# songweige/rich-text-to-image

Measured on NVIDIA H100. Metric: denoising steps/sec, higher is better.
Workload: dtype f16

## Files before the change

### include/rtti_b200.h

```cpp
#ifndef RTTI_B200_H
#define RTTI_B200_H

#ifdef __cplusplus
extern "C" {
#endif

#define RTTI_OK 0
#define RTTI_ERR_ARG (-1)
#define RTTI_ERR_SHAPE (-2)
#define RTTI_ERR_ALIGN (-3)
#define RTTI_ERR_ARCH (-4)
#define RTTI_ERR_CUDA (-5)

int rtti_version(void);
int rtti_arch_ok(void);

int rtti_attn_fwd(const void* q, const void* k, const void* v, void* o, int batch, int heads, int head_dim,
                  int n_q, int n_k, long long q_bs, long long q_rs, long long k_bs, long long k_rs,
                  long long v_bs, long long v_rs, long long o_bs, long long o_rs, float scale,
                  const int* qk_src, const int* word_pos, const float* font_size, int n_fs,
                  unsigned long long fs_batch_mask, float* pbar_accum, const int* cap_slot, float* lse,
                  void* stream);

int rtti_attn_probs_mean_accum(const void* q, const void* k, const float* lse, float* accum, int heads,
                               int head_dim, int n_q, int n_k, long long q_rs, long long k_rs, float scale,
                               void* stream);

long long rtti_groupnorm_workspace_elems(int batch, int hw, int c, int groups);
int rtti_groupnorm_silu_fwd(const void* x, const void* chan_bias, const void* gamma, const void* beta, void* y,
                            float* workspace, int batch, int hw, int c, int groups, float eps, int apply_silu,
                            void* stream);

int rtti_add_bias_f16(const void* a, const void* b, const void* bias, void* out, long long rows, int c, void* stream);

int rtti_layernorm_fwd(const void* x, const void* gamma, const void* beta, void* y, int rows, int c, float eps,
                       void* stream);

int rtti_ff_geglu_fwd(const void* x, const void* w, const void* bias, void* y, long long m, int n, int k, void* stream);

int rtti_add_bias_layernorm_fwd(const void* a, const void* resid, const void* bias, const void* gamma, const void* beta,
                                void* h_out, void* y, int rows, int c, float eps, void* stream);

int rtti_geglu_fwd(const void* proj, void* y, int rows, int inner, void* stream);

int rtti_region_blend_cfg(const void* eps_uncond, const void* const* eps_region, const float* masks,
                          int n_regions, long long n, float guidance, void* eps_out, const void* latents,
                          void* latents_out, float dt_sigma, void* stream);

long long rtti_color_loss_workspace_elems(int n_colors, long long hw);
int rtti_color_loss_fwd_bwd(const float* decoded, const float* masks, const float* target_rgb, int n_colors,
                            long long hw, float* loss_out, float* grad_decoded, float* workspace, void* stream);

int rtti_latent_guidance_update(const void* latents, const float* grad, const float* atten_all, float weight,
                                void* latents_out, long long n, void* stream);

int rtti_bg_inject_blend(const void* latents, const void* latents_ref, const float* mask, void* out,
                         long long n, void* stream);

int rtti_predict_x0(const void* x_t, const void* eps, float alpha, void* x0, long long n, void* stream);

long long rtti_gn32_workspace_elems(int batch, int hw, int c, int groups);
int rtti_gn32_silu_fwd(const float* x, const float* chan_bias, const float* gamma, const float* beta, float* y,
                       float* mean_rstd, float* workspace, int batch, int hw, int c, int groups, float eps,
                       int apply_silu, void* stream);
int rtti_gn32_silu_bwd(const float* x, const float* chan_bias, const float* dz, const float* gamma, const float* beta,
                       const float* mean_rstd, float* dx, float* workspace, int batch, int hw, int c, int groups,
                       int apply_silu, void* stream);
int rtti_add_bias_f32(const float* a, const float* b, const float* bias, float* out, long long rows, int c,
                      void* stream);

int rtti_gather_blend_step(const void* const* peer_slots, void* const* peer_flags, int world, int rank,
                           const int* slot_owner, int n_slots, int n_regions, const float* masks, long long n,
                           float guidance, void* eps_out, const void* latents, void* latents_out,
                           const void* latents_ref, void* latents_ref_out, float dt_sigma, unsigned int step_id,
                           void* stream);

int rtti_gn32_silu_fwd_striped(const float* x, const float* chan_bias, const float* gamma, const float* beta, float* y,
                               float* mean_rstd, float* workspace, int hw_local, long long hw_total, int c, int groups,
                               float eps, int apply_silu, void* const* peer_sums, void* const* peer_flags, int world,
                               int rank, unsigned int seq, void* stream);
int rtti_gn32_silu_bwd_striped(const float* x, const float* chan_bias, const float* dz, const float* gamma,
                               const float* beta, const float* mean_rstd, float* dx, float* workspace, int hw_local,
                               long long hw_total, int c, int groups, int apply_silu, void* const* peer_sums,
                               void* const* peer_flags, int world, int rank, unsigned int seq, void* stream);
int rtti_halo_exchange(float* pad_local, float* pad_up, float* pad_down, int rows, long long row_elems,
                       void* flags_local, void* flags_up, void* flags_down, unsigned int seq, void* stream);
int rtti_peer_seq_advance(void* flags_a, unsigned int da, void* flags_b, unsigned int db, void* stream);

int rtti_peer_push(const void* src, long long src_row_stride_bytes, int rows, int row_bytes, void* const* dst,
                   void* const* dst_flags, int n_dst, void* flags_local, unsigned int seq, void* stream);
int rtti_peer_wait(void* flags_local, unsigned int seq, void* stream);

#ifdef __cplusplus
}
#endif
#endif
```

### rich-text-to-image_b200/_lib.py

```python
import ctypes
import os

PKG_DIR = os.path.dirname(os.path.abspath(__file__))
LIB_PATH = os.path.join(PKG_DIR, "librtti_b200.so")

RTTI_OK = 0
_ERRORS = {
    -1: "RTTI_ERR_ARG (null pointer / out-of-range argument)",
    -2: "RTTI_ERR_SHAPE (unsupported shape)",
    -3: "RTTI_ERR_ALIGN (pointer or stride alignment)",
    -4: "RTTI_ERR_ARCH (device is not sm_90)",
    -5: "RTTI_ERR_CUDA (CUDA runtime/driver error)",
}

c_void_p, c_int, c_ll, c_float, c_ull = ctypes.c_void_p, ctypes.c_int, ctypes.c_longlong, ctypes.c_float, ctypes.c_ulonglong
P_int = ctypes.POINTER(ctypes.c_int)

SIGNATURES = {
    "rtti_version": (c_int, []),
    "rtti_arch_ok": (c_int, []),
    "rtti_attn_fwd": (c_int, [c_void_p] * 4 + [c_int] * 5 + [c_ll] * 8 + [c_float, P_int, c_void_p, c_void_p, c_int,
                                                                         c_ull, c_void_p, P_int, c_void_p, c_void_p]),
    "rtti_attn_probs_mean_accum": (c_int, [c_void_p] * 4 + [c_int] * 4 + [c_ll] * 2 + [c_float, c_void_p]),
    "rtti_groupnorm_workspace_elems": (c_ll, [c_int] * 4),
    "rtti_groupnorm_silu_fwd": (c_int, [c_void_p] * 6 + [c_int] * 4 + [c_float, c_int, c_void_p]),
    "rtti_add_bias_f16": (c_int, [c_void_p] * 4 + [c_ll, c_int, c_void_p]),
    "rtti_layernorm_fwd": (c_int, [c_void_p] * 4 + [c_int, c_int, c_float, c_void_p]),
    "rtti_add_bias_layernorm_fwd": (c_int, [c_void_p] * 7 + [c_int, c_int, c_float, c_void_p]),
    "rtti_ff_geglu_fwd": (c_int, [c_void_p] * 4 + [c_ll, c_int, c_int, c_void_p]),
    "rtti_geglu_fwd": (c_int, [c_void_p, c_void_p, c_int, c_int, c_void_p]),
    "rtti_region_blend_cfg": (c_int, [c_void_p, ctypes.POINTER(c_void_p), c_void_p, c_int, c_ll, c_float, c_void_p,
                                      c_void_p, c_void_p, c_float, c_void_p]),
    "rtti_color_loss_workspace_elems": (c_ll, [c_int, c_ll]),
    "rtti_color_loss_fwd_bwd": (c_int, [c_void_p] * 3 + [c_int, c_ll] + [c_void_p] * 4),
    "rtti_latent_guidance_update": (c_int, [c_void_p] * 3 + [c_float, c_void_p, c_ll, c_void_p]),
    "rtti_bg_inject_blend": (c_int, [c_void_p] * 4 + [c_ll, c_void_p]),
    "rtti_predict_x0": (c_int, [c_void_p, c_void_p, c_float, c_void_p, c_ll, c_void_p]),
    "rtti_gn32_workspace_elems": (c_ll, [c_int] * 4),
    "rtti_gn32_silu_fwd": (c_int, [c_void_p] * 7 + [c_int] * 4 + [c_float, c_int, c_void_p]),
    "rtti_gn32_silu_bwd": (c_int, [c_void_p] * 8 + [c_int] * 4 + [c_int, c_void_p]),
    "rtti_add_bias_f32": (c_int, [c_void_p] * 4 + [c_ll, c_int, c_void_p]),
    "rtti_gather_blend_step": (c_int, [ctypes.POINTER(c_void_p), ctypes.POINTER(c_void_p), c_int, c_int, P_int, c_int, c_int,
                                       c_void_p, c_ll, c_float, c_void_p, c_void_p, c_void_p, c_void_p, c_void_p, c_float,
                                       ctypes.c_uint, c_void_p]),
    "rtti_gn32_silu_fwd_striped": (c_int, [c_void_p] * 7 + [c_int, c_ll, c_int, c_int, c_float, c_int,
                                           ctypes.POINTER(c_void_p), ctypes.POINTER(c_void_p), c_int, c_int, ctypes.c_uint,
                                           c_void_p]),
    "rtti_gn32_silu_bwd_striped": (c_int, [c_void_p] * 8 + [c_int, c_ll, c_int, c_int, c_int,
                                           ctypes.POINTER(c_void_p), ctypes.POINTER(c_void_p), c_int, c_int, ctypes.c_uint,
                                           c_void_p]),
    "rtti_halo_exchange": (c_int, [c_void_p] * 3 + [c_int, c_ll] + [c_void_p] * 3 + [ctypes.c_uint, c_void_p]),
    "rtti_peer_seq_advance": (c_int, [c_void_p, ctypes.c_uint, c_void_p, ctypes.c_uint, c_void_p]),
    "rtti_peer_push": (c_int, [c_void_p, c_ll, c_int, c_int, ctypes.POINTER(c_void_p), ctypes.POINTER(c_void_p), c_int,
                               c_void_p, ctypes.c_uint, c_void_p]),
    "rtti_peer_wait": (c_int, [c_void_p, ctypes.c_uint, c_void_p]),
}

_lib = None


class RttiError(RuntimeError):
    pass


def load():
    global _lib
    if _lib is not None:
        return _lib
    if not os.path.exists(LIB_PATH):
        raise RttiError(
            f"{LIB_PATH} not found: build it with `python -c 'import __graft_entry__ as g; g.build()'` "
            "(the rtti_b200 product path has no CPU/PyTorch fallback)")
    lib = ctypes.CDLL(LIB_PATH)
    for name, (res, args) in SIGNATURES.items():
        fn = getattr(lib, name)
        fn.restype = res
        fn.argtypes = args
    _lib = lib
    return lib


def check(rc, what):
    if rc != RTTI_OK:
        raise RttiError(f"{what} failed: {_ERRORS.get(rc, rc)}")
```

### rich-text-to-image_b200/csrc/vae_kernels.cu

```cuda
#include "peer_sync.cuh"
#include "rtti_internal.h"

namespace rtti {

struct GN32Plan { int nvec, rowlanes, threads, chunks, rows_per_chunk; };

static GN32Plan gn32_plan(int batch, int hw, int c) {
  GN32Plan p;
  p.nvec = c / 4;
  p.rowlanes = p.nvec >= 256 ? 1 : (256 / p.nvec);
  p.threads = p.nvec * p.rowlanes;
  int want = (132 * 8 + batch - 1) / batch;
  int maxc = (hw + p.rowlanes * 8 - 1) / (p.rowlanes * 8);
  if (maxc < 1) maxc = 1;
  p.chunks = want < maxc ? want : maxc;
  if (p.chunks < 1) p.chunks = 1;
  p.rows_per_chunk = (hw + p.chunks - 1) / p.chunks;
  p.rows_per_chunk = ((p.rows_per_chunk + p.rowlanes - 1) / p.rowlanes) * p.rowlanes;
  p.chunks = (hw + p.rows_per_chunk - 1) / p.rows_per_chunk;
  return p;
}

__device__ __forceinline__ float sigmoidf_(float x) { return 1.f / (1.f + __expf(-x)); }

// ... 65 lines not shown
  }
#pragma unroll
  for (int i = 0; i < 4; ++i) {
    sm[((size_t)rl * c + vec * 4 + i) * 2] = a[i];
    sm[((size_t)rl * c + vec * 4 + i) * 2 + 1] = q[i];
  }
  __syncthreads();
  for (int g = threadIdx.x; g < groups; g += blockDim.x) {
    float s0 = 0.f, s1 = 0.f;
    for (int l = 0; l < rowlanes; ++l)
      for (int ch = g * cpg; ch < (g + 1) * cpg; ++ch) {
        s0 += sm[((size_t)l * c + ch) * 2];
        s1 += sm[((size_t)l * c + ch) * 2 + 1];
      }
    float* o = ws + (((size_t)b * chunks + chunk) * groups + g) * 2;
    o[0] = s0; o[1] = s1;
  }
}

template <int MODE>
__global__ void gn32_finalize_kernel(const float* __restrict__ ws, float* __restrict__ out, int groups, int chunks,
                                     float n, float eps) {
  const int b = blockIdx.y;
  const int g = blockIdx.x * (blockDim.x >> 5) + (threadIdx.x >> 5);
  const int lane = threadIdx.x & 31;
  if (g >= groups) return;
  float s0 = 0.f, s1 = 0.f;
  for (int k = lane; k < chunks; k += 32) {
    const float* o = ws + (((size_t)b * chunks + k) * groups + g) * 2;
    s0 += o[0]; s1 += o[1];
  }
#pragma unroll
  for (int o = 16; o > 0; o >>= 1) {
    s0 += __shfl_xor_sync(0xffffffffu, s0, o);
    s1 += __shfl_xor_sync(0xffffffffu, s1, o);
  }
  if (lane == 0) {
    float* d = out + ((size_t)b * groups + g) * 2;
    if (MODE == 0) {
      const float mean = s0 / n;
      const float var = fmaxf(s1 / n - mean * mean, 0.f);
      d[0] = mean; d[1] = rsqrtf(var + eps);
    } else {
      d[0] = s0 / n; d[1] = s1 / n;
    }
  }
}

template <int MODE>
__global__ void gn32_apply_kernel(const float* __restrict__ x, const float* __restrict__ cbias,
                                  const float* __restrict__ dz,
                                  const float* __restrict__ gamma, const float* __restrict__ beta,
                                  const float* __restrict__ mean_rstd, const float* __restrict__ c12,
                                  float* __restrict__ out, int hw, int c, int groups, int nvec, int rowlanes,
                                  int rows_per_chunk, int silu) {
  const int b = blockIdx.y, chunk = blockIdx.x;
  const int vec = threadIdx.x % nvec, rl = threadIdx.x / nvec;
  const int cpg = c / groups;
  float ga[4], be[4], mu[4], rs[4], c1[4], c2[4];
  float cb[4] = {0.f, 0.f, 0.f, 0.f};
  if (cbias) { const float4 c4 = *reinterpret_cast<const float4*>(cbias + vec * 4); cb[0] = c4.x; cb[1] = c4.y; cb[2] = c4.z; cb[3] = c4.w; }
  const float4 g4 = *reinterpret_cast<const float4*>(gamma + vec * 4);
  const float4 b4 = *reinterpret_cast<const float4*>(beta + vec * 4);
  ga[0] = g4.x; ga[1] = g4.y; ga[2] = g4.z; ga[3] = g4.w;
  be[0] = b4.x; be[1] = b4.y; be[2] = b4.z; be[3] = b4.w;
#pragma unroll
  for (int i = 0; i < 4; ++i) {
    const int g = (vec * 4 + i) / cpg;
    mu[i] = mean_rstd[((size_t)b * groups + g) * 2];
    rs[i] = mean_rstd[((size_t)b * groups + g) * 2 + 1];
    if (MODE == 1) { c1[i] = c12[((size_t)b * groups + g) * 2]; c2[i] = c12[((size_t)b * groups + g) * 2 + 1]; }
  }
  const int r0 = chunk * rows_per_chunk, r1 = min(hw, r0 + rows_per_chunk);
  const size_t base = ((size_t)b * hw) * c + vec * 4;
  auto apply = [&](const float4& xv, const float4& dv) -> float4 {
    const float xs[4] = {xv.x + cb[0], xv.y + cb[1], xv.z + cb[2], xv.w + cb[3]};
    float o[4];
    if (MODE == 0) {
#pragma unroll
      for (int i = 0; i < 4; ++i) {
        const float y = fmaf((xs[i] - mu[i]) * rs[i], ga[i], be[i]);
        o[i] = silu ? y * sigmoidf_(y) : y;
      }
    } else {
      const float ds[4] = {dv.x, dv.y, dv.z, dv.w};
#pragma unroll
      for (int i = 0; i < 4; ++i) {
        const float xh = (xs[i] - mu[i]) * rs[i];
        float dy = ds[i];
        if (silu) {
          const float y = fmaf(xh, ga[i], be[i]);
          const float s = sigmoidf_(y);
          dy *= s * (1.f + y * (1.f - s));
        }
        o[i] = rs[i] * (dy * ga[i] - c1[i] - xh * c2[i]);
      }
    }
    return make_float4(o[0], o[1], o[2], o[3]);
  };
  int r = r0 + rl;
  for (; r + 3 * rowlanes < r1; r += 4 * rowlanes) {
    float4 xv[4], dv[4];
#pragma unroll
    for (int u = 0; u < 4; ++u) {
      xv[u] = *reinterpret_cast<const float4*>(x + base + (size_t)(r + u * rowlanes) * c);
      if (MODE == 1) dv[u] = *reinterpret_cast<const float4*>(dz + base + (size_t)(r + u * rowlanes) * c);
    }
#pragma unroll
    for (int u = 0; u < 4; ++u)
      *reinterpret_cast<float4*>(out + base + (size_t)(r + u * rowlanes) * c) = apply(xv[u], dv[u]);
  }
  for (; r < r1; r += rowlanes) {
    const float4 xv = *reinterpret_cast<const float4*>(x + base + (size_t)r * c);
    float4 dv = xv;
    if (MODE == 1) dv = *reinterpret_cast<const float4*>(dz + base + (size_t)r * c);
    *reinterpret_cast<float4*>(out + base + (size_t)r * c) = apply(xv, dv);
  }
}

static int gn32_check(const void* a, const void* b_, const void* c_, const void* d, int batch, int hw, int c, int groups) {
  if (!a || !b_ || !c_ || !d) return RTTI_ERR_ARG;
  if (batch < 1 || hw < 1 || groups < 1) return RTTI_ERR_ARG;
  if (c % 4 != 0 || c % groups != 0 || c / 4 > 1024) return RTTI_ERR_SHAPE;
  if (((uintptr_t)a | (uintptr_t)b_ | (uintptr_t)c_ | (uintptr_t)d) & 15) return RTTI_ERR_ALIGN;
  return RTTI_OK;
}

struct PeerSums {
  float* sums[PEER_MAX_WORLD];
  unsigned int* flags[PEER_MAX_WORLD];
  int world, rank;
  unsigned int seq;
};

template <int MODE>
__global__ void __launch_bounds__(1024) gn32_finalize_peer_kernel(const float* __restrict__ ws, float* __restrict__ out,
                                                                  const PeerSums pp, int groups, int chunks,
                                                                  float n_total, float eps) {
  const int g = threadIdx.x >> 5, lane = threadIdx.x & 31;
  const unsigned int seq = pp.seq + *reinterpret_cast<const volatile unsigned int*>(pp.flags[pp.rank] + 8);
  const int par = (int)(seq & 1u);
  if (g < groups) {
    float s0 = 0.f, s1 = 0.f;
    for (int k = lane; k < chunks; k += 32) {
      const float* o = ws + ((size_t)k * groups + g) * 2;
      s0 += o[0]; s1 += o[1];
    }
#pragma unroll
    for (int o = 16; o > 0; o >>= 1) {
      s0 += __shfl_xor_sync(0xffffffffu, s0, o);
      s1 += __shfl_xor_sync(0xffffffffu, s1, o);
    }
    if (lane == 0) {
      float* mine = pp.sums[pp.rank] + (size_t)par * 2 * groups;
      mine[2 * g] = s0; mine[2 * g + 1] = s1;
    }
  }
  __syncthreads();
  if (threadIdx.x == 0) {
    __threadfence_system();
    st_release_sys(pp.flags[pp.rank], seq);
  }
  if (threadIdx.x < pp.world && threadIdx.x != pp.rank) {
    if (!wait_seq(pp.flags[threadIdx.x], seq)) pp.flags[pp.rank][1] = 0xDEADu;
  }
  __syncthreads();
  if (g < groups && lane == 0) {
    float t0 = 0.f, t1 = 0.f;
    for (int r = 0; r < pp.world; ++r) {
// ... 1 lines not shown
      t0 += ld_volatile_f32(p + 2 * g);
      t1 += ld_volatile_f32(p + 2 * g + 1);
    }
    float* d = out + (size_t)g * 2;
    if (MODE == 0) {
      const float mean = t0 / n_total;
      const float var = fmaxf(t1 / n_total - mean * mean, 0.f);
      d[0] = mean; d[1] = rsqrtf(var + eps);
    } else {
      d[0] = t0 / n_total; d[1] = t1 / n_total;
    }
  }
}

static int fill_peer_sums(PeerSums& pp, void* const* peer_sums, void* const* peer_flags, int world, int rank,
                          unsigned int seq) {
  if (!peer_sums || !peer_flags) return RTTI_ERR_ARG;
  if (world < 1 || world > PEER_MAX_WORLD || rank < 0 || rank >= world) return RTTI_ERR_ARG;
  for (int r = 0; r < world; ++r) {
    if (!peer_sums[r] || !peer_flags[r]) return RTTI_ERR_ARG;
    if (((uintptr_t)peer_sums[r] | (uintptr_t)peer_flags[r]) & 3) return RTTI_ERR_ALIGN;
    pp.sums[r] = (float*)peer_sums[r];
    pp.flags[r] = (unsigned int*)peer_flags[r];
  }
  pp.world = world; pp.rank = rank; pp.seq = seq;
  return RTTI_OK;
}

}

using namespace rtti;

extern "C" long long rtti_gn32_workspace_elems(int batch, int hw, int c, int groups) {
  if (batch < 1 || hw < 1 || c < 4 || groups < 1) return 0;
  const GN32Plan p = gn32_plan(batch, hw, c);
  return (long long)batch * p.chunks * groups * 2 + (long long)batch * groups * 2;
}

extern "C" int rtti_gn32_silu_fwd(const float* x, const float* chan_bias, const float* gamma, const float* beta, float* y, float* mean_rstd,
                                  float* workspace, int batch, int hw, int c, int groups, float eps, int apply_silu,
                                  void* stream) {
  int rc = gn32_check(x, gamma, beta, y, batch, hw, c, groups);
  if (rc != RTTI_OK) return rc;
  if (!mean_rstd || !workspace) return RTTI_ERR_ARG;
  const GN32Plan p = gn32_plan(batch, hw, c);
  const size_t smem = (size_t)p.rowlanes * c * 2 * sizeof(float);
  if (smem > 48 * 1024) return RTTI_ERR_SHAPE;
  cudaStream_t st = (cudaStream_t)stream;
  dim3 grid(p.chunks, batch);
  gn32_partial_kernel<0><<<grid, p.threads, smem, st>>>(x, chan_bias, nullptr, gamma, beta, nullptr, workspace, hw, c, groups,
                                                        p.nvec, p.rowlanes, p.rows_per_chunk, p.chunks, 0);
  gn32_finalize_kernel<0><<<dim3((groups + 7) / 8, batch), 256, 0, st>>>(workspace, mean_rstd, groups, p.chunks,
                                                                         (float)hw * (float)(c / groups), eps);
  gn32_apply_kernel<0><<<grid, p.threads, 0, st>>>(x, chan_bias, nullptr, gamma, beta, mean_rstd, nullptr, y, hw, c, groups,
                                                   p.nvec, p.rowlanes, p.rows_per_chunk, apply_silu);
  return cudaGetLastError() == cudaSuccess ? RTTI_OK : RTTI_ERR_CUDA;
}

extern "C" int rtti_gn32_silu_bwd(const float* x, const float* chan_bias, const float* dz, const float* gamma, const float* beta,
                                  const float* mean_rstd, float* dx, float* workspace, int batch, int hw, int c,
                                  int groups, int apply_silu, void* stream) {
  int rc = gn32_check(x, gamma, beta, dx, batch, hw, c, groups);
  if (rc != RTTI_OK) return rc;
  if (!dz || !mean_rstd || !workspace || ((uintptr_t)dz & 15)) return RTTI_ERR_ARG;
  const GN32Plan p = gn32_plan(batch, hw, c);
  const size_t smem = (size_t)p.rowlanes * c * 2 * sizeof(float);
  if (smem > 48 * 1024) return RTTI_ERR_SHAPE;
  cudaStream_t st = (cudaStream_t)stream;
  dim3 grid(p.chunks, batch);
  float* c12 = workspace + (size_t)batch * p.chunks * groups * 2;
  gn32_partial_kernel<1><<<grid, p.threads, smem, st>>>(x, chan_bias, dz, gamma, beta, mean_rstd, workspace, hw, c, groups, p.nvec,
                                                        p.rowlanes, p.rows_per_chunk, p.chunks, apply_silu);
  gn32_finalize_kernel<1><<<dim3((groups + 7) / 8, batch), 256, 0, st>>>(workspace, c12, groups, p.chunks,
                                                                         (float)hw * (float)(c / groups), 0.f);
  gn32_apply_kernel<1><<<grid, p.threads, 0, st>>>(x, chan_bias, dz, gamma, beta, mean_rstd, c12, dx, hw, c, groups, p.nvec,
                                                   p.rowlanes, p.rows_per_chunk, apply_silu);
  return cudaGetLastError() == cudaSuccess ? RTTI_OK : RTTI_ERR_CUDA;
}


extern "C" int rtti_gn32_silu_fwd_striped(const float* x, const float* chan_bias, const float* gamma, const float* beta,
                                          float* y, float* mean_rstd, float* workspace, int hw_local, long long hw_total,
                                          int c, int groups, float eps, int apply_silu, void* const* peer_sums,
                                          void* const* peer_flags, int world, int rank, unsigned int seq, void* stream) {
  int rc = gn32_check(x, gamma, beta, y, 1, hw_local, c, groups);
  if (rc != RTTI_OK) return rc;
  if (!mean_rstd || !workspace || hw_total < hw_local) return RTTI_ERR_ARG;
  if (groups > 32) return RTTI_ERR_SHAPE;
  PeerSums pp{};
  rc = fill_peer_sums(pp, peer_sums, peer_flags, world, rank, seq);
  if (rc != RTTI_OK) return rc;
  const GN32Plan p = gn32_plan(1, hw_local, c);
  const size_t smem = (size_t)p.rowlanes * c * 2 * sizeof(float);
  if (smem > 48 * 1024) return RTTI_ERR_SHAPE;
  cudaStream_t st = (cudaStream_t)stream;
  dim3 grid(p.chunks, 1);
  gn32_partial_kernel<0><<<grid, p.threads, smem, st>>>(x, chan_bias, nullptr, gamma, beta, nullptr, workspace, hw_local, c,
                                                        groups, p.nvec, p.rowlanes, p.rows_per_chunk, p.chunks, 0);
  gn32_finalize_peer_kernel<0><<<1, 32 * groups, 0, st>>>(workspace, mean_rstd, pp, groups, p.chunks,
                                                          (float)hw_total * (float)(c / groups), eps);
  gn32_apply_kernel<0><<<grid, p.threads, 0, st>>>(x, chan_bias, nullptr, gamma, beta, mean_rstd, nullptr, y, hw_local, c,
                                                   groups, p.nvec, p.rowlanes, p.rows_per_chunk, apply_silu);
  return cudaGetLastError() == cudaSuccess ? RTTI_OK : RTTI_ERR_CUDA;
}

extern "C" int rtti_gn32_silu_bwd_striped(const float* x, const float* chan_bias, const float* dz, const float* gamma,
                                          const float* beta, const float* mean_rstd, float* dx, float* workspace,
                                          int hw_local, long long hw_total, int c, int groups, int apply_silu,
                                          void* const* peer_sums, void* const* peer_flags, int world, int rank,
                                          unsigned int seq, void* stream) {
  int rc = gn32_check(x, gamma, beta, dx, 1, hw_local, c, groups);
  if (rc != RTTI_OK) return rc;
  if (!dz || !mean_rstd || !workspace || ((uintptr_t)dz & 15) || hw_total < hw_local) return RTTI_ERR_ARG;
  if (groups > 32) return RTTI_ERR_SHAPE;
  PeerSums pp{};
  rc = fill_peer_sums(pp, peer_sums, peer_flags, world, rank, seq);
  if (rc != RTTI_OK) return rc;
  const GN32Plan p = gn32_plan(1, hw_local, c);
  const size_t smem = (size_t)p.rowlanes * c * 2 * sizeof(float);
  if (smem > 48 * 1024) return RTTI_ERR_SHAPE;
  cudaStream_t st = (cudaStream_t)stream;
  dim3 grid(p.chunks, 1);
  float* c12 = workspace + (size_t)p.chunks * groups * 2;
  gn32_partial_kernel<1><<<grid, p.threads, smem, st>>>(x, chan_bias, dz, gamma, beta, mean_rstd, workspace, hw_local, c,
                                                        groups, p.nvec, p.rowlanes, p.rows_per_chunk, p.chunks, apply_silu);
  gn32_finalize_peer_kernel<1><<<1, 32 * groups, 0, st>>>(workspace, c12, pp, groups, p.chunks,
                                                          (float)hw_total * (float)(c / groups), 0.f);
  gn32_apply_kernel<1><<<grid, p.threads, 0, st>>>(x, chan_bias, dz, gamma, beta, mean_rstd, c12, dx, hw_local, c, groups,
                                                   p.nvec, p.rowlanes, p.rows_per_chunk, apply_silu);
  return cudaGetLastError() == cudaSuccess ? RTTI_OK : RTTI_ERR_CUDA;
}

__global__ void add_bias_f32_kernel(const float* __restrict__ a, const float* __restrict__ b,
                                    const float* __restrict__ bias, float* __restrict__ out, long long nvec, int cvec) {
  for (long long i = (long long)blockIdx.x * blockDim.x + threadIdx.x; i < nvec; i += (long long)gridDim.x * blockDim.x) {
    const float4 x = reinterpret_cast<const float4*>(a)[i];
    const float4 y = reinterpret_cast<const float4*>(b)[i];
    float4 z = make_float4(0.f, 0.f, 0.f, 0.f);
    if (bias) z = reinterpret_cast<const float4*>(bias)[i % cvec];
    reinterpret_cast<float4*>(out)[i] = make_float4(x.x + y.x + z.x, x.y + y.y + z.y, x.z + y.z + z.z, x.w + y.w + z.w);
  }
}

extern "C" int rtti_add_bias_f32(const float* a, const float* b, const float* bias, float* out, long long rows, int c,
                                 void* stream) {
  if (!a || !b || !out || rows < 1 || c < 4) return RTTI_ERR_ARG;
  if (c % 4 != 0) return RTTI_ERR_SHAPE;
  if (((uintptr_t)a | (uintptr_t)b | (uintptr_t)out | (uintptr_t)bias) & 15) return RTTI_ERR_ALIGN;
  const long long nvec = rows * (c / 4);
  long long blocks = (nvec + 255) / 256;
  if (blocks > 132 * 16) blocks = 132 * 16;
  add_bias_f32_kernel<<<(int)blocks, 256, 0, (cudaStream_t)stream>>>(a, b, bias, out, nvec, c / 4);
  return cudaGetLastError() == cudaSuccess ? RTTI_OK : RTTI_ERR_CUDA;
}
```

### rich-text-to-image_b200/ops.py

```python
import ctypes
import math

import torch

from . import _lib

_F16 = torch.float16

LAUNCHES = 0
FUSED_FF_GEGLU = True
PROFILE = None


def _count(n):
    global LAUNCHES
    LAUNCHES += n


_raw_stream = getattr(torch._C, "_cuda_getCurrentRawStream", None)


def _stream():
    if _raw_stream is not None:
        return ctypes.c_void_p(_raw_stream(torch.cuda.current_device()))
# ... 255 lines not shown

def gather_blend_step(peer_slot_ptrs, peer_flag_ptrs, rank, slot_owner, n_regions, masks, guidance, latents, latents_ref,
                      dt_sigma, step_id):
    lib = _lib.load()
    world = len(peer_slot_ptrs)
    n = latents.numel()
    _req(latents, _F16, "latents"); _req(masks, torch.float32, "masks")
    eps = torch.empty_like(latents)
    lat_out = torch.empty_like(latents)
    ref_out = torch.empty_like(latents_ref) if latents_ref is not None else None
    slots = (ctypes.c_void_p * world)(*peer_slot_ptrs)
    flags = (ctypes.c_void_p * world)(*peer_flag_ptrs)
    rc = lib.rtti_gather_blend_step(slots, flags, world, rank, _int_array(slot_owner), len(slot_owner), n_regions,
                                    _ptr(masks), n, float(guidance), _ptr(eps), _ptr(latents), _ptr(lat_out),
                                    _ptr(latents_ref), _ptr(ref_out), float(dt_sigma), int(step_id), _stream())
    _lib.check(rc, "rtti_gather_blend_step")
    _count(1)
    return eps, lat_out, ref_out


_gn32_ws = {}


_gn32_ws_elems = {}


def _gn32_workspace(x, groups):
    B, HW, C = x.shape
    n = _gn32_ws_elems.get((B, HW, C, groups))
    if n is None:
        n = _gn32_ws_elems[(B, HW, C, groups)] = _lib.load().rtti_gn32_workspace_elems(B, HW, C, groups)
    key = (x.device.index, _stream().value)
    ws = _gn32_ws.get(key)
    if ws is None or ws.numel() < n:
        ws = torch.empty(max(n, 1 << 18), dtype=torch.float32, device=x.device)
        _gn32_ws[key] = ws
    return ws


def gn32_silu_fwd(x, gamma, beta, groups, eps, silu, chan_bias=None):
    lib = _lib.load()
    _req(x, torch.float32, "x"); _req(gamma, torch.float32, "gamma"); _req(beta, torch.float32, "beta")
    assert x.dim() == 3 and x.is_contiguous()
    B, HW, C = x.shape
    y = torch.empty_like(x)
    stats = torch.empty(B, groups, 2, dtype=torch.float32, device=x.device)
    rc = lib.rtti_gn32_silu_fwd(_ptr(x), _ptr(chan_bias), _ptr(gamma), _ptr(beta), _ptr(y), _ptr(stats), _ptr(_gn32_workspace(x, groups)),
                                B, HW, C, groups, float(eps), 1 if silu else 0, _stream())
    _lib.check(rc, "rtti_gn32_silu_fwd")
    _count(3)
    return y, stats


def gn32_silu_bwd(x, dz, gamma, beta, stats, groups, silu, chan_bias=None):
    lib = _lib.load()
    _req(x, torch.float32, "x"); _req(dz, torch.float32, "dz")
    assert x.is_contiguous() and dz.is_contiguous() and dz.shape == x.shape
    B, HW, C = x.shape
    dx = torch.empty_like(x)
    rc = lib.rtti_gn32_silu_bwd(_ptr(x), _ptr(chan_bias), _ptr(dz), _ptr(gamma), _ptr(beta), _ptr(stats), _ptr(dx),
                                _ptr(_gn32_workspace(x, groups)), B, HW, C, groups, 1 if silu else 0, _stream())
    _lib.check(rc, "rtti_gn32_silu_bwd")
    _count(3)
    return dx


def gn32_silu_fwd_striped(x, gamma, beta, groups, eps, silu, hw_total, peers, seq, chan_bias=None, out=None):
    lib = _lib.load()
    _req(x, torch.float32, "x"); _req(gamma, torch.float32, "gamma"); _req(beta, torch.float32, "beta")
    assert x.dim() == 3 and x.shape[0] == 1 and x.is_contiguous()
    _, HW, C = x.shape
    y = torch.empty_like(x) if out is None else out
    assert y.is_contiguous() and y.numel() == x.numel() and y.dtype == torch.float32
    stats = torch.empty(1, groups, 2, dtype=torch.float32, device=x.device)
    rc = lib.rtti_gn32_silu_fwd_striped(_ptr(x), _ptr(chan_bias), _ptr(gamma), _ptr(beta), _ptr(y), _ptr(stats),
                                        _ptr(_gn32_workspace(x, groups)), HW, int(hw_total), C, groups, float(eps),
                                        1 if silu else 0, peers.sum_ptrs, peers.gn_flag_ptrs, peers.world, peers.rank,
                                        int(seq), _stream())
    _lib.check(rc, "rtti_gn32_silu_fwd_striped")
    _count(3)
    return y, stats


def gn32_silu_bwd_striped(x, dz, gamma, beta, stats, groups, silu, hw_total, peers, seq, chan_bias=None, out=None):
    lib = _lib.load()
    _req(x, torch.float32, "x"); _req(dz, torch.float32, "dz")
    assert x.is_contiguous() and dz.is_contiguous() and dz.numel() == x.numel() and x.shape[0] == 1
    _, HW, C = x.shape
    dx = torch.empty_like(x) if out is None else out
    assert dx.is_contiguous() and dx.numel() == x.numel() and dx.dtype == torch.float32
    rc = lib.rtti_gn32_silu_bwd_striped(_ptr(x), _ptr(chan_bias), _ptr(dz), _ptr(gamma), _ptr(beta), _ptr(stats), _ptr(dx),
                                        _ptr(_gn32_workspace(x, groups)), HW, int(hw_total), C, groups, 1 if silu else 0,
                                        peers.sum_ptrs, peers.gn_flag_ptrs, peers.world, peers.rank, int(seq), _stream())
    _lib.check(rc, "rtti_gn32_silu_bwd_striped")
    _count(3)
    return dx


def halo_exchange(pad, pad_ptr_up, pad_ptr_down, flags_local, flags_up, flags_down, seq):
    lib = _lib.load()
    _req(pad, torch.float32, "pad")
    assert pad.dim() == 3 and pad.is_contiguous()
    rows = pad.shape[0] - 2
    rc = lib.rtti_halo_exchange(_ptr(pad), ctypes.c_void_p(pad_ptr_up or 0), ctypes.c_void_p(pad_ptr_down or 0), rows,
                                pad.shape[1] * pad.shape[2], ctypes.c_void_p(flags_local),
                                ctypes.c_void_p(flags_up or 0), ctypes.c_void_p(flags_down or 0), int(seq), _stream())
    _lib.check(rc, "rtti_halo_exchange")
    _count(1)


def peer_seq_advance(flags_a, da, flags_b=0, db=0):
    lib = _lib.load()
    rc = lib.rtti_peer_seq_advance(ctypes.c_void_p(flags_a or 0), int(da), ctypes.c_void_p(flags_b or 0), int(db), _stream())
    _lib.check(rc, "rtti_peer_seq_advance")
    _count(1)


def peer_push(src, dst_ptrs, dst_flag_ptrs, flags_local, seq):
    lib = _lib.load()
    _req(src, _F16, "src")
    assert src.dim() == 2 and src.stride(1) == 1
    rc = lib.rtti_peer_push(_ptr(src), src.stride(0) * 2, src.shape[0], src.shape[1] * 2, dst_ptrs, dst_flag_ptrs,
                            len(dst_ptrs), ctypes.c_void_p(flags_local), int(seq), _stream())
    _lib.check(rc, "rtti_peer_push")
    _count(1)


def peer_wait(flags_local, seq):
    lib = _lib.load()
    _lib.check(lib.rtti_peer_wait(ctypes.c_void_p(flags_local), int(seq), _stream()), "rtti_peer_wait")
    _count(1)


def add_bias_f32(a, b, bias=None, out=None):
    lib = _lib.load()
    _req(a, torch.float32, "a"); _req(b, torch.float32, "b")
    assert a.is_contiguous() and b.is_contiguous() and a.shape == b.shape
    C = a.shape[-1]
    if out is None:
        out = torch.empty_like(a)
    _lib.check(lib.rtti_add_bias_f32(_ptr(a), _ptr(b), _ptr(bias), _ptr(out), a.numel() // C, C, _stream()), "rtti_add_bias_f32")
    _count(1)
    return out


def add_bias_f16(a, b, bias=None, out=None):
    lib = _lib.load()
    _req(a, _F16, "a"); _req(b, _F16, "b")
    assert a.is_contiguous() and b.is_contiguous() and a.shape == b.shape
    C = a.shape[-1]
    if out is None:
        out = torch.empty_like(a)
    _lib.check(lib.rtti_add_bias_f16(_ptr(a), _ptr(b), _ptr(bias), _ptr(out), a.numel() // C, C, _stream()), "rtti_add_bias_f16")
    _count(1)
    return out
```

### rich-text-to-image_b200/vae_guidance.py

```python
import math

import torch
import torch.nn.functional as F

from . import ops

_conv_bwd = torch.ops.aten.convolution_backward


class _Tape(list):
    pass


def _nchw(x, H, W):
    return x.view(x.shape[0], H, W, x.shape[2]).permute(0, 3, 1, 2)


def _cl(y):
    B, C, H, W = y.shape
    y = y.permute(0, 2, 3, 1)
    if not y.is_contiguous():
        y = y.contiguous()
    return y.view(B, H * W, C), H, W


def _conv_f(conv, x, H, W, with_bias=True):
    y = F.conv2d(_nchw(x, H, W), conv.weight, conv.bias if with_bias else None, conv.stride, conv.padding)
    return _cl(y)[0]


class DecoderFwdBwd:

    def __init__(self, vae):
        self.vae = vae
        self.groups = vae.config.norm_num_groups
        self._dummies = {}

    def _gn_f(self, norm, x, silu, tape, chan_bias=None):
        y, stats = ops.gn32_silu_fwd(x, norm.weight, norm.bias, self.groups, norm.eps, silu, chan_bias=chan_bias)
        tape.append(("gn", norm, x, stats, silu, chan_bias))
        return y

    def _gn_b(self, rec, g):
        _, norm, x, stats, silu, chan_bias = rec
        return ops.gn32_silu_bwd(x, g.contiguous(), norm.weight, norm.bias, stats, self.groups, silu, chan_bias=chan_bias)

    def _dummy(self, shape, dev):
        k = (tuple(shape), str(dev))
        if k not in self._dummies:
            self._dummies[k] = torch.empty(shape, dtype=torch.float32, device=dev, memory_format=torch.channels_last)
        return self._dummies[k]

    def _conv_b(self, conv, g, cin, H, W):
        g4 = _nchw(g, H, W)
        gi, _, _ = _conv_bwd(g4, self._dummy((g.shape[0], cin, H, W), g.device), conv.weight, None, list(conv.stride),
                             list(conv.padding), [1, 1], False, [0, 0], 1, [True, False, False])
        return _cl(gi)[0]

    def _resnet_f(self, r, x, H, W, tape):
        h = self._gn_f(r.norm1, x, True, tape)
        h = _conv_f(r.conv1, h, H, W, with_bias=False)
        h = self._gn_f(r.norm2, h, True, tape, chan_bias=r.conv1.bias)
        h = _conv_f(r.conv2, h, H, W, with_bias=False)
        sc = _conv_f(r.conv_shortcut, x, H, W) if r.conv_shortcut is not None else x
        tape.append(("res", r, H, W))
        return ops.add_bias_f32(sc, h, r.conv2.bias)

    def _resnet_b(self, tape, g):
        _, r, H, W = tape.pop()
        cin, cout = r.conv1.in_channels, r.conv1.out_channels
        dh = self._conv_b(r.conv2, g, cout, H, W)
        dh = self._gn_b(tape.pop(), dh)
        dh = self._conv_b(r.conv1, dh, cin, H, W)
        dx = self._gn_b(tape.pop(), dh)
        if r.conv_shortcut is not None:
            return ops.add_bias_f32(dx, self._conv_b(r.conv_shortcut, g, cin, H, W))
        return ops.add_bias_f32(dx, g.contiguous())

    def _attn_f(self, a, x, tape):
        B, T, C = x.shape
        hn = self._gn_f(a.group_norm, x, False, tape)
        q = F.linear(hn, a.to_q.weight, a.to_q.bias)
        k = F.linear(hn, a.to_k.weight, a.to_k.bias)
        v = F.linear(hn, a.to_v.weight, a.to_v.bias)
        scale = 1.0 / math.sqrt(C)
        p = torch.softmax(torch.bmm(q * scale, k.transpose(1, 2)), dim=-1)
        o = torch.bmm(p, v)
        tape.append(("attn", a, hn, q, k, v, p, scale))
        return x + F.linear(o, a.to_out[0].weight, a.to_out[0].bias)

    def _attn_b(self, tape, g):
        _, a, hn, q, k, v, p, scale = tape.pop()
        do = g @ a.to_out[0].weight
        dv = torch.bmm(p.transpose(1, 2), do)
        dp = torch.bmm(do, v.transpose(1, 2))
        ds = torch._softmax_backward_data(dp, p, -1, p.dtype)
        dq = torch.bmm(ds, k * scale)
        dk = torch.bmm(ds.transpose(1, 2), q * scale)
        dhn = dq @ a.to_q.weight + dk @ a.to_k.weight + dv @ a.to_v.weight
        return g + self._gn_b(tape.pop(), dhn)

    def forward(self, z):
        vae, d = self.vae, self.vae.decoder
        prev = torch.backends.cuda.matmul.allow_tf32
        torch.backends.cuda.matmul.allow_tf32 = True
        try:
            tape = _Tape()
            B, _, H, W = z.shape
            x = z.permute(0, 2, 3, 1).contiguous().view(B, H * W, -1)
            x = _conv_f(vae.post_quant_conv, x, H, W)
            x = _conv_f(d.conv_in, x, H, W)
            x = self._resnet_f(d.mid_block.resnets[0], x, H, W, tape)
            x = self._attn_f(d.mid_block.attentions[0], x, tape)
            x = self._resnet_f(d.mid_block.resnets[1], x, H, W, tape)
            for blk in d.up_blocks:
                for r in blk.resnets:
                    x = self._resnet_f(r, x, H, W, tape)
                if blk.upsamplers is not None:
                    C = x.shape[2]
                    x = x.view(B, H, 1, W, 1, C).expand(B, H, 2, W, 2, C).reshape(B, 4 * H * W, C)
                    H, W = 2 * H, 2 * W
                    x = _conv_f(blk.upsamplers[0].conv, x, H, W)
                    tape.append(("up", blk.upsamplers[0].conv, H, W, C))
            x = self._gn_f(d.conv_norm_out, x, True, tape)
            y = _conv_f(d.conv_out, x, H, W)
            tape.append(("out", H, W))
            self.tape = tape
            return _nchw(y, H, W)
        finally:
            torch.backends.cuda.matmul.allow_tf32 = prev

    def backward(self, grad_image):
        vae, d = self.vae, self.vae.decoder
        prev = torch.backends.cuda.matmul.allow_tf32
        torch.backends.cuda.matmul.allow_tf32 = True
        try:
            tape = self.tape
            _, H, W = tape.pop()
            B = grad_image.shape[0]
            g = grad_image.permute(0, 2, 3, 1).contiguous().view(B, H * W, -1)
            g = self._conv_b(d.conv_out, g, d.conv_out.in_channels, H, W)
            g = self._gn_b(tape.pop(), g)
            for blk in reversed(d.up_blocks):
                if blk.upsamplers is not None:
                    _, conv, H, W, C = tape.pop()
                    g = self._conv_b(conv, g, C, H, W)
                    H, W = H // 2, W // 2
                    g = g.view(B, H, 2, W, 2, C).sum(dim=(2, 4)).reshape(B, H * W, C)
                for _ in blk.resnets:
                    g = self._resnet_b(tape, g)
            g = self._resnet_b(tape, g)
            g = self._attn_b(tape, g)
            g = self._resnet_b(tape, g)
            g = self._conv_b(d.conv_in, g, d.conv_in.in_channels, H, W)
            g = self._conv_b(vae.post_quant_conv, g, vae.post_quant_conv.in_channels, H, W)
            self.tape = None
            return g.view(B, H, W, -1).permute(0, 3, 1, 2).contiguous()
        finally:
            torch.backends.cuda.matmul.allow_tf32 = prev


def default_engine(vae):
    eng = getattr(vae, "_fwd_bwd", None)
    if eng is None:
        eng = vae._fwd_bwd = DecoderFwdBwd(vae)
    return eng


def image_and_latent_grad(vae, z, grad_fn, engine=None):
    from .vae import AutoencoderKLDecoder
    if isinstance(vae, AutoencoderKLDecoder):
        eng = engine if engine is not None else default_engine(vae)
        img = eng.forward(z)
        return eng.backward(grad_fn(img))
    z = z.detach().requires_grad_(True)
    with torch.enable_grad():
        img = vae.decode_tensor(z)
    img.backward(grad_fn(img.detach()))
    return z.grad


class GuidanceGraph:

    def __init__(self, engine):
        self.engine = engine
        self.calls = 0
        self.graph = None
        self.launches = 0

    def _run(self, z, masks, tgt):
        img = self.engine.forward(z)
        loss, g = ops.color_loss_fwd_bwd(img[0].contiguous(), masks, tgt)
        return loss, self.engine.backward(g[None])

    def __call__(self, z, masks, tgt):
        self.calls += 1
        if self.calls == 1:
            return self._run(z, masks, tgt)
        if self.graph is None:
            self.z, self.masks, self.tgt = z.clone(), masks.clone(), tgt.clone()
            torch.cuda.synchronize(z.device)
# ... 12 lines not shown
```

Measured before the change: 3.521.

## Fold nearest-upsample into phase-decomposed 2x2 conv and fuse residual add into GN backward

Replaces the VAE decoder's nearest-neighbor 2x upsample followed by a 3x3 conv with a polyphase 2x2 conv on the low-resolution input. Four output phases are computed as 4x channels and then interleaved, with a matching scatter kernel and conv backward for the gradient. This cuts conv FLOPs by about 2.25x and avoids materializing the upsampled activation. Separately, the resnet residual gradient add is fused into the GroupNorm backward apply kernel through a new addend argument, dropping one elementwise pass. The costs are extra interleave/scatter passes over a padded (h+1)x(w+1) grid and a cached fp32 phase filter built in double precision.

```diff
diff --git a/include/rtti_b200.h b/include/rtti_b200.h
--- a/include/rtti_b200.h
+++ b/include/rtti_b200.h
@@ -64,8 +64,11 @@
                        float* mean_rstd, float* workspace, int batch, int hw, int c, int groups, float eps,
                        int apply_silu, void* stream);
 int rtti_gn32_silu_bwd(const float* x, const float* chan_bias, const float* dz, const float* gamma, const float* beta,
-                       const float* mean_rstd, float* dx, float* workspace, int batch, int hw, int c, int groups,
-                       int apply_silu, void* stream);
+                       const float* mean_rstd, const float* addend, float* dx, float* workspace, int batch, int hw,
+                       int c, int groups, int apply_silu, void* stream);
+int rtti_upsample_phase_interleave(const float* y4, const float* bias, float* out, int batch, int h, int w, int c,
+                                   void* stream);
+int rtti_upsample_phase_scatter(const float* g, float* dy4, int batch, int h, int w, int c, void* stream);
 int rtti_add_bias_f32(const float* a, const float* b, const float* bias, float* out, long long rows, int c,
                       void* stream);
 
diff --git a/rich-text-to-image_b200/_lib.py b/rich-text-to-image_b200/_lib.py
--- a/rich-text-to-image_b200/_lib.py
+++ b/rich-text-to-image_b200/_lib.py
@@ -38,8 +38,10 @@
     "rtti_predict_x0": (c_int, [c_void_p, c_void_p, c_float, c_void_p, c_ll, c_void_p]),
     "rtti_gn32_workspace_elems": (c_ll, [c_int] * 4),
     "rtti_gn32_silu_fwd": (c_int, [c_void_p] * 7 + [c_int] * 4 + [c_float, c_int, c_void_p]),
-    "rtti_gn32_silu_bwd": (c_int, [c_void_p] * 8 + [c_int] * 4 + [c_int, c_void_p]),
+    "rtti_gn32_silu_bwd": (c_int, [c_void_p] * 9 + [c_int] * 4 + [c_int, c_void_p]),
     "rtti_add_bias_f32": (c_int, [c_void_p] * 4 + [c_ll, c_int, c_void_p]),
+    "rtti_upsample_phase_interleave": (c_int, [c_void_p] * 3 + [c_int] * 4 + [c_void_p]),
+    "rtti_upsample_phase_scatter": (c_int, [c_void_p] * 2 + [c_int] * 4 + [c_void_p]),
     "rtti_gather_blend_step": (c_int, [ctypes.POINTER(c_void_p), ctypes.POINTER(c_void_p), c_int, c_int, P_int, c_int, c_int,
                                        c_void_p, c_ll, c_float, c_void_p, c_void_p, c_void_p, c_void_p, c_void_p, c_float,
                                        ctypes.c_uint, c_void_p]),
diff --git a/rich-text-to-image_b200/csrc/vae_kernels.cu b/rich-text-to-image_b200/csrc/vae_kernels.cu
--- a/rich-text-to-image_b200/csrc/vae_kernels.cu
+++ b/rich-text-to-image_b200/csrc/vae_kernels.cu
@@ -141,6 +141,7 @@
                                   const float* __restrict__ dz,
                                   const float* __restrict__ gamma, const float* __restrict__ beta,
                                   const float* __restrict__ mean_rstd, const float* __restrict__ c12,
+                                  const float* __restrict__ addend,
                                   float* __restrict__ out, int hw, int c, int groups, int nvec, int rowlanes,
                                   int rows_per_chunk, int silu) {
   const int b = blockIdx.y, chunk = blockIdx.x;
@@ -187,6 +188,14 @@
     }
     return make_float4(o[0], o[1], o[2], o[3]);
   };
+  auto store = [&](int row, float4 v) {
+    const size_t off = base + (size_t)row * c;
+    if (MODE == 1 && addend) {
+      const float4 a = *reinterpret_cast<const float4*>(addend + off);
+      v.x += a.x; v.y += a.y; v.z += a.z; v.w += a.w;
+    }
+    *reinterpret_cast<float4*>(out + off) = v;
+  };
   int r = r0 + rl;
   for (; r + 3 * rowlanes < r1; r += 4 * rowlanes) {
     float4 xv[4], dv[4];
@@ -196,14 +205,13 @@
       if (MODE == 1) dv[u] = *reinterpret_cast<const float4*>(dz + base + (size_t)(r + u * rowlanes) * c);
     }
 #pragma unroll
-    for (int u = 0; u < 4; ++u)
-      *reinterpret_cast<float4*>(out + base + (size_t)(r + u * rowlanes) * c) = apply(xv[u], dv[u]);
+    for (int u = 0; u < 4; ++u) store(r + u * rowlanes, apply(xv[u], dv[u]));
   }
   for (; r < r1; r += rowlanes) {
     const float4 xv = *reinterpret_cast<const float4*>(x + base + (size_t)r * c);
     float4 dv = xv;
     if (MODE == 1) dv = *reinterpret_cast<const float4*>(dz + base + (size_t)r * c);
-    *reinterpret_cast<float4*>(out + base + (size_t)r * c) = apply(xv, dv);
+    store(r, apply(xv, dv));
   }
 }
 
@@ -311,17 +319,18 @@
                                                         p.nvec, p.rowlanes, p.rows_per_chunk, p.chunks, 0);
   gn32_finalize_kernel<0><<<dim3((groups + 7) / 8, batch), 256, 0, st>>>(workspace, mean_rstd, groups, p.chunks,
                                                                          (float)hw * (float)(c / groups), eps);
-  gn32_apply_kernel<0><<<grid, p.threads, 0, st>>>(x, chan_bias, nullptr, gamma, beta, mean_rstd, nullptr, y, hw, c, groups,
-                                                   p.nvec, p.rowlanes, p.rows_per_chunk, apply_silu);
+  gn32_apply_kernel<0><<<grid, p.threads, 0, st>>>(x, chan_bias, nullptr, gamma, beta, mean_rstd, nullptr, nullptr, y, hw, c,
+                                                   groups, p.nvec, p.rowlanes, p.rows_per_chunk, apply_silu);
   return cudaGetLastError() == cudaSuccess ? RTTI_OK : RTTI_ERR_CUDA;
 }
 
 extern "C" int rtti_gn32_silu_bwd(const float* x, const float* chan_bias, const float* dz, const float* gamma, const float* beta,
-                                  const float* mean_rstd, float* dx, float* workspace, int batch, int hw, int c,
-                                  int groups, int apply_silu, void* stream) {
+                                  const float* mean_rstd, const float* addend, float* dx, float* workspace, int batch,
+                                  int hw, int c, int groups, int apply_silu, void* stream) {
   int rc = gn32_check(x, gamma, beta, dx, batch, hw, c, groups);
   if (rc != RTTI_OK) return rc;
   if (!dz || !mean_rstd || !workspace || ((uintptr_t)dz & 15)) return RTTI_ERR_ARG;
+  if ((uintptr_t)addend & 15) return RTTI_ERR_ALIGN;
   const GN32Plan p = gn32_plan(batch, hw, c);
   const size_t smem = (size_t)p.rowlanes * c * 2 * sizeof(float);
   if (smem > 48 * 1024) return RTTI_ERR_SHAPE;
@@ -332,8 +341,8 @@
                                                         p.rowlanes, p.rows_per_chunk, p.chunks, apply_silu);
   gn32_finalize_kernel<1><<<dim3((groups + 7) / 8, batch), 256, 0, st>>>(workspace, c12, groups, p.chunks,
                                                                          (float)hw * (float)(c / groups), 0.f);
-  gn32_apply_kernel<1><<<grid, p.threads, 0, st>>>(x, chan_bias, dz, gamma, beta, mean_rstd, c12, dx, hw, c, groups, p.nvec,
-                                                   p.rowlanes, p.rows_per_chunk, apply_silu);
+  gn32_apply_kernel<1><<<grid, p.threads, 0, st>>>(x, chan_bias, dz, gamma, beta, mean_rstd, c12, addend, dx, hw, c, groups,
+                                                   p.nvec, p.rowlanes, p.rows_per_chunk, apply_silu);
   return cudaGetLastError() == cudaSuccess ? RTTI_OK : RTTI_ERR_CUDA;
 }
 
@@ -358,8 +367,8 @@
                                                         groups, p.nvec, p.rowlanes, p.rows_per_chunk, p.chunks, 0);
   gn32_finalize_peer_kernel<0><<<1, 32 * groups, 0, st>>>(workspace, mean_rstd, pp, groups, p.chunks,
                                                           (float)hw_total * (float)(c / groups), eps);
-  gn32_apply_kernel<0><<<grid, p.threads, 0, st>>>(x, chan_bias, nullptr, gamma, beta, mean_rstd, nullptr, y, hw_local, c,
-                                                   groups, p.nvec, p.rowlanes, p.rows_per_chunk, apply_silu);
+  gn32_apply_kernel<0><<<grid, p.threads, 0, st>>>(x, chan_bias, nullptr, gamma, beta, mean_rstd, nullptr, nullptr, y, hw_local,
+                                                   c, groups, p.nvec, p.rowlanes, p.rows_per_chunk, apply_silu);
   return cudaGetLastError() == cudaSuccess ? RTTI_OK : RTTI_ERR_CUDA;
 }
 
@@ -385,8 +394,8 @@
                                                         groups, p.nvec, p.rowlanes, p.rows_per_chunk, p.chunks, apply_silu);
   gn32_finalize_peer_kernel<1><<<1, 32 * groups, 0, st>>>(workspace, c12, pp, groups, p.chunks,
                                                           (float)hw_total * (float)(c / groups), 0.f);
-  gn32_apply_kernel<1><<<grid, p.threads, 0, st>>>(x, chan_bias, dz, gamma, beta, mean_rstd, c12, dx, hw_local, c, groups,
-                                                   p.nvec, p.rowlanes, p.rows_per_chunk, apply_silu);
+  gn32_apply_kernel<1><<<grid, p.threads, 0, st>>>(x, chan_bias, dz, gamma, beta, mean_rstd, c12, nullptr, dx, hw_local, c,
+                                                   groups, p.nvec, p.rowlanes, p.rows_per_chunk, apply_silu);
   return cudaGetLastError() == cudaSuccess ? RTTI_OK : RTTI_ERR_CUDA;
 }
 
@@ -412,3 +421,71 @@
   add_bias_f32_kernel<<<(int)blocks, 256, 0, (cudaStream_t)stream>>>(a, b, bias, out, nvec, c / 4);
   return cudaGetLastError() == cudaSuccess ? RTTI_OK : RTTI_ERR_CUDA;
 }
+
+
+__global__ void upsample_phase_interleave_kernel(const float* __restrict__ y4, const float* __restrict__ bias,
+                                                 float* __restrict__ out, long long nvec, int h, int w, int cvec) {
+  const int H = 2 * h, W = 2 * w;
+  for (long long i = (long long)blockIdx.x * blockDim.x + threadIdx.x; i < nvec; i += (long long)gridDim.x * blockDim.x) {
+    const int cv = (int)(i % cvec);
+    long long pix = i / cvec;
+    const int x = (int)(pix % W); pix /= W;
+    const int y = (int)(pix % H);
+    const long long b = pix / H;
+    const int a = y & 1, bb = x & 1;
+    const long long src = ((b * (h + 1) + (y >> 1) + a) * (w + 1) + (x >> 1) + bb) * (4LL * cvec) + (2 * a + bb) * cvec + cv;
+    float4 v = reinterpret_cast<const float4*>(y4)[src];
+    if (bias) {
+      const float4 z = reinterpret_cast<const float4*>(bias)[cv];
+      v.x += z.x; v.y += z.y; v.z += z.z; v.w += z.w;
+    }
+    reinterpret_cast<float4*>(out)[i] = v;
+  }
+}
+
+__global__ void upsample_phase_scatter_kernel(const float* __restrict__ g, float* __restrict__ dy4, long long nvec, int h,
+                                              int w, int cvec) {
+  for (long long i = (long long)blockIdx.x * blockDim.x + threadIdx.x; i < nvec; i += (long long)gridDim.x * blockDim.x) {
+    const int cv = (int)(i % (4 * cvec));
+    long long pix = i / (4 * cvec);
+    const int q = (int)(pix % (w + 1)); pix /= (w + 1);
+    const int p = (int)(pix % (h + 1));
+    const long long b = pix / (h + 1);
+    const int k = cv / cvec, a = k >> 1, bb = k & 1;
+    const int li = p - a, lj = q - bb;
+    float4 v = make_float4(0.f, 0.f, 0.f, 0.f);
+    if (li >= 0 && li < h && lj >= 0 && lj < w)
+      v = reinterpret_cast<const float4*>(g)[((b * 2 * h + 2 * li + a) * (2LL * w) + 2 * lj + bb) * cvec + cv % cvec];
+    reinterpret_cast<float4*>(dy4)[i] = v;
+  }
+}
+
+static int upsample_phase_check(const void* a, const void* b, int batch, int h, int w, int c) {
+  if (!a || !b || batch < 1 || h < 1 || w < 1 || c < 4) return RTTI_ERR_ARG;
+  if (c % 4 != 0) return RTTI_ERR_SHAPE;
+  if (((uintptr_t)a | (uintptr_t)b) & 15) return RTTI_ERR_ALIGN;
+  return RTTI_OK;
+}
+
+static int elementwise_blocks(long long nvec) {
+  const long long blocks = (nvec + 255) / 256;
+  return (int)(blocks < 132 * 16 ? blocks : 132 * 16);
+}
+
+extern "C" int rtti_upsample_phase_interleave(const float* y4, const float* bias, float* out, int batch, int h, int w, int c,
+                                              void* stream) {
+  int rc = upsample_phase_check(y4, out, batch, h, w, c);
+  if (rc != RTTI_OK) return rc;
+  if ((uintptr_t)bias & 15) return RTTI_ERR_ALIGN;
+  const long long nvec = (long long)batch * 4 * h * w * (c / 4);
+  upsample_phase_interleave_kernel<<<elementwise_blocks(nvec), 256, 0, (cudaStream_t)stream>>>(y4, bias, out, nvec, h, w, c / 4);
+  return cudaGetLastError() == cudaSuccess ? RTTI_OK : RTTI_ERR_CUDA;
+}
+
+extern "C" int rtti_upsample_phase_scatter(const float* g, float* dy4, int batch, int h, int w, int c, void* stream) {
+  int rc = upsample_phase_check(g, dy4, batch, h, w, c);
+  if (rc != RTTI_OK) return rc;
+  const long long nvec = (long long)batch * (h + 1) * (w + 1) * c;
+  upsample_phase_scatter_kernel<<<elementwise_blocks(nvec), 256, 0, (cudaStream_t)stream>>>(g, dy4, nvec, h, w, c / 4);
+  return cudaGetLastError() == cudaSuccess ? RTTI_OK : RTTI_ERR_CUDA;
+}
diff --git a/rich-text-to-image_b200/ops.py b/rich-text-to-image_b200/ops.py
--- a/rich-text-to-image_b200/ops.py
+++ b/rich-text-to-image_b200/ops.py
@@ -331,14 +331,17 @@
     return y, stats
 
 
-def gn32_silu_bwd(x, dz, gamma, beta, stats, groups, silu, chan_bias=None):
+def gn32_silu_bwd(x, dz, gamma, beta, stats, groups, silu, chan_bias=None, addend=None):
     lib = _lib.load()
     _req(x, torch.float32, "x"); _req(dz, torch.float32, "dz")
     assert x.is_contiguous() and dz.is_contiguous() and dz.shape == x.shape
+    if addend is not None:
+        _req(addend, torch.float32, "addend")
+        assert addend.is_contiguous() and addend.shape == x.shape
     B, HW, C = x.shape
     dx = torch.empty_like(x)
-    rc = lib.rtti_gn32_silu_bwd(_ptr(x), _ptr(chan_bias), _ptr(dz), _ptr(gamma), _ptr(beta), _ptr(stats), _ptr(dx),
-                                _ptr(_gn32_workspace(x, groups)), B, HW, C, groups, 1 if silu else 0, _stream())
+    rc = lib.rtti_gn32_silu_bwd(_ptr(x), _ptr(chan_bias), _ptr(dz), _ptr(gamma), _ptr(beta), _ptr(stats), _ptr(addend),
+                                _ptr(dx), _ptr(_gn32_workspace(x, groups)), B, HW, C, groups, 1 if silu else 0, _stream())
     _lib.check(rc, "rtti_gn32_silu_bwd")
     _count(3)
     return dx
@@ -423,6 +426,32 @@
     return out
 
 
+def upsample_phase_interleave(y4, bias, h, w):
+    lib = _lib.load()
+    _req(y4, torch.float32, "y4")
+    B, n, C4 = y4.shape
+    assert y4.is_contiguous() and n == (h + 1) * (w + 1) and C4 % 4 == 0
+    C = C4 // 4
+    if bias is not None:
+        _req(bias, torch.float32, "bias"); assert bias.is_contiguous() and bias.numel() == C
+    out = torch.empty(B, 4 * h * w, C, dtype=torch.float32, device=y4.device)
+    _lib.check(lib.rtti_upsample_phase_interleave(_ptr(y4), _ptr(bias), _ptr(out), B, h, w, C, _stream()),
+               "rtti_upsample_phase_interleave")
+    _count(1)
+    return out
+
+
+def upsample_phase_scatter(g, h, w):
+    lib = _lib.load()
+    _req(g, torch.float32, "g")
+    B, n, C = g.shape
+    assert g.is_contiguous() and n == 4 * h * w
+    dy4 = torch.empty(B, (h + 1) * (w + 1), 4 * C, dtype=torch.float32, device=g.device)
+    _lib.check(lib.rtti_upsample_phase_scatter(_ptr(g), _ptr(dy4), B, h, w, C, _stream()), "rtti_upsample_phase_scatter")
+    _count(1)
+    return dy4
+
+
 def add_bias_f16(a, b, bias=None, out=None):
     lib = _lib.load()
     _req(a, _F16, "a"); _req(b, _F16, "b")
diff --git a/rich-text-to-image_b200/vae_guidance.py b/rich-text-to-image_b200/vae_guidance.py
--- a/rich-text-to-image_b200/vae_guidance.py
+++ b/rich-text-to-image_b200/vae_guidance.py
@@ -6,6 +6,8 @@
 from . import ops
 
 _conv_bwd = torch.ops.aten.convolution_backward
+
+_PHASE_TAPS = (((1., 0., 0.), (0., 1., 1.)), ((1., 1., 0.), (0., 0., 1.)))
 
 
 class _Tape(list):
@@ -35,15 +37,17 @@
         self.vae = vae
         self.groups = vae.config.norm_num_groups
         self._dummies = {}
+        self._wphase = {}
 
     def _gn_f(self, norm, x, silu, tape, chan_bias=None):
         y, stats = ops.gn32_silu_fwd(x, norm.weight, norm.bias, self.groups, norm.eps, silu, chan_bias=chan_bias)
         tape.append(("gn", norm, x, stats, silu, chan_bias))
         return y
 
-    def _gn_b(self, rec, g):
+    def _gn_b(self, rec, g, addend=None):
         _, norm, x, stats, silu, chan_bias = rec
-        return ops.gn32_silu_bwd(x, g.contiguous(), norm.weight, norm.bias, stats, self.groups, silu, chan_bias=chan_bias)
+        return ops.gn32_silu_bwd(x, g.contiguous(), norm.weight, norm.bias, stats, self.groups, silu, chan_bias=chan_bias,
+                                 addend=addend)
 
     def _dummy(self, shape, dev):
         k = (tuple(shape), str(dev))
@@ -55,6 +59,25 @@
         g4 = _nchw(g, H, W)
         gi, _, _ = _conv_bwd(g4, self._dummy((g.shape[0], cin, H, W), g.device), conv.weight, None, list(conv.stride),
                              list(conv.padding), [1, 1], False, [0, 0], 1, [True, False, False])
+        return _cl(gi)[0]
+
+    def _phase_filter(self, conv):
+        hit = self._wphase.get(id(conv))
+        if hit is None or hit[0] is not conv:
+            w = conv.weight.double()
+            taps = torch.tensor(_PHASE_TAPS, dtype=w.dtype, device=w.device)
+            wf = torch.einsum("atk,bul,oikl->aboitu", taps, taps, w).reshape(4 * w.shape[0], w.shape[1], 2, 2)
+            hit = self._wphase[id(conv)] = (conv, wf.float().contiguous(memory_format=torch.channels_last))
+        return hit[1]
+
+    def _upsample_f(self, conv, x, H, W):
+        y4 = F.conv2d(_nchw(x, H, W), self._phase_filter(conv), None, 1, 1)
+        return ops.upsample_phase_interleave(_cl(y4)[0], conv.bias, H, W)
+
+    def _upsample_b(self, conv, g, H, W, C):
+        dy4 = ops.upsample_phase_scatter(g.contiguous(), H, W)
+        gi, _, _ = _conv_bwd(_nchw(dy4, H + 1, W + 1), self._dummy((g.shape[0], C, H, W), g.device), self._phase_filter(conv),
+                             None, [1, 1], [1, 1], [1, 1], False, [0, 0], 1, [True, False, False])
         return _cl(gi)[0]
 
     def _resnet_f(self, r, x, H, W, tape):
@@ -72,10 +95,8 @@
         dh = self._conv_b(r.conv2, g, cout, H, W)
         dh = self._gn_b(tape.pop(), dh)
         dh = self._conv_b(r.conv1, dh, cin, H, W)
-        dx = self._gn_b(tape.pop(), dh)
-        if r.conv_shortcut is not None:
-            return ops.add_bias_f32(dx, self._conv_b(r.conv_shortcut, g, cin, H, W))
-        return ops.add_bias_f32(dx, g.contiguous())
+        sc = self._conv_b(r.conv_shortcut, g, cin, H, W) if r.conv_shortcut is not None else g.contiguous()
+        return self._gn_b(tape.pop(), dh, addend=sc)
 
     def _attn_f(self, a, x, tape):
         B, T, C = x.shape
@@ -118,10 +139,9 @@
                     x = self._resnet_f(r, x, H, W, tape)
                 if blk.upsamplers is not None:
                     C = x.shape[2]
-                    x = x.view(B, H, 1, W, 1, C).expand(B, H, 2, W, 2, C).reshape(B, 4 * H * W, C)
+                    x = self._upsample_f(blk.upsamplers[0].conv, x, H, W)
+                    tape.append(("up", blk.upsamplers[0].conv, H, W, C))
                     H, W = 2 * H, 2 * W
-                    x = _conv_f(blk.upsamplers[0].conv, x, H, W)
-                    tape.append(("up", blk.upsamplers[0].conv, H, W, C))
             x = self._gn_f(d.conv_norm_out, x, True, tape)
             y = _conv_f(d.conv_out, x, H, W)
             tape.append(("out", H, W))
@@ -144,9 +164,7 @@
             for blk in reversed(d.up_blocks):
                 if blk.upsamplers is not None:
                     _, conv, H, W, C = tape.pop()
-                    g = self._conv_b(conv, g, C, H, W)
-                    H, W = H // 2, W // 2
-                    g = g.view(B, H, 2, W, 2, C).sum(dim=(2, 4)).reshape(B, H * W, C)
+                    g = self._upsample_b(conv, g, H, W, C)
                 for _ in blk.resnets:
                     g = self._resnet_b(tape, g)
             g = self._resnet_b(tape, g)
```

Result: faster. 3.711, median of 6 (+5.4%).
